# RichExplor/VIL_Fusion

Hardware: AMD Instinct MI355X
Metric: sliding-window solve iters/sec (10 KF, ~5.5k factors) @1/2/4/8 GPU vs CPU (higher is better)
Workload: dtype f64

## Files before the change

### include/vilfusion.h

```cpp
#ifndef VILFUSION_H
#define VILFUSION_H

#include <stdint.h>

#ifdef __cplusplus
extern "C" {
#endif

#define VILF_MAX_FRAMES 11
#define VILF_MAX_FEATURES 1000
#define VILF_PRIOR_MAX_DIM 160
#define VILF_PRIOR_MAX_BLOCKS 24

#define VILF_OK 0
#define VILF_ERR_INVALID_ARGUMENT (-1)
#define VILF_ERR_DEVICE (-2)
#define VILF_ERR_UNSUPPORTED (-3)
#define VILF_ERR_NO_GPU (-4)
#define VILF_SOLVER_ABNORMAL 1

#define VILF_MARGIN_OLD 0
#define VILF_MARGIN_SECOND_NEW 1

#define VILF_TERM_NO_CONVERGENCE 0
// ... 197 lines not shown
    double rel_q[4], rel_t[3];
    int n_edge_ds, n_surf_ds;
    int n_edge_factors[2];
    int n_surf_factors[2];
    int iterations[2];
    double final_cost[2];
    int map_edge_size, map_surf_size;
} vilf_scan2map_result;
int vilf_scan2map_step(vilf_handle *h, const float *edge_xyzi, int n_edge, const float *surf_xyzi, int n_surf,
                       vilf_scan2map_result *res);
int vilf_scan2map_get_map(vilf_handle *h, int which , float *xyzi_out, int capacity, int *n_out);
int vilf_scan2map_set_pose(vilf_handle *h, const double pose_qt[7], const double pose_last_qt[7]);

int vilf_scan2map_batch_create(vilf_handle *h, int n_streams, int cap_scan_edge, int cap_scan_surf, int cap_map_edge, int cap_map_surf);
int vilf_scan2map_batch_init(vilf_handle *h, int stream, const float *edge_xyzi, int n_edge, const float *surf_xyzi, int n_surf,
                             const double *pose_qt, const double *pose_last_qt);
int vilf_scan2map_batch_set_scan(vilf_handle *h, int stream, const float *edge_xyzi, int n_edge, const float *surf_xyzi, int n_surf);
int vilf_scan2map_batch_copy_stream(vilf_handle *h, int src, int dst);
int vilf_scan2map_batch_step(vilf_handle *h, int sync);
int vilf_scan2map_batch_snapshot(vilf_handle *h);
int vilf_scan2map_batch_rewind(vilf_handle *h);
int vilf_scan2map_batch_results(vilf_handle *h, int first, int n, vilf_scan2map_result *res);
int vilf_scan2map_batch_get_map(vilf_handle *h, int stream, int which, float *xyzi_out, int capacity, int *n_out);

int vilf_lidar_extract_features(vilf_handle *h, const float *xyzi, int n_points, int n_scans, double min_range, double max_range,
                                double edge_threshold, float *edge_xyzi_out, int cap_edge, int *n_edge,
                                float *surf_xyzi_out, int cap_surf, int *n_surf);
int vilf_feature_depth(vilf_handle *h, const float *depth_cloud_xyzi, int n_points, const float *features_xyz, int n_features, float *depth_out);
#ifdef __cplusplus
}
#endif
#endif
```

### vil_fusion_amd/csrc/vilf_s2m.hip

```cpp
#include <hip/hip_runtime.h>
#include <cstring>
#include <string.h>
#include <cmath>
#include <climits>
#include <algorithm>
#include <utility>
#include "vilf_sort.hpp"
#include "vilf_internal.hpp"
#include "vilf_device.hpp"

#ifdef VILF_STAMPS
__device__ long long s2m_dbg[9 * 32];
#define S2M_STAMP_WG 1500
#define S2M_STAMP(kid, i, cond) do { if (blockIdx.x == S2M_STAMP_WG && threadIdx.x == 0 && (cond)) s2m_dbg[(kid) * 32 + (i)] = __builtin_readcyclecounter(); } while (0)
extern "C" int vilf_debug_stamps_s2m(long long *out288) { return hipMemcpyFromSymbol(out288, HIP_SYMBOL(s2m_dbg), sizeof(long long) * 9 * 32) == hipSuccess ? 0 : -1; }
#define S2M_ACC_DECL long long acc_t[8] = {0, 0, 0, 0, 0, 0, 0, 0}; long long acc_last = __builtin_readcyclecounter();
#define S2M_ACC(i) do { const long long now_ = __builtin_readcyclecounter(); acc_t[i] += now_ - acc_last; acc_last = now_; } while (0)
#define S2M_ACC_OUT(kid) do { if (blockIdx.x == S2M_STAMP_WG && threadIdx.x == 0) for (int i_ = 0; i_ < 8; i_++) s2m_dbg[(kid) * 32 + 16 + i_] = acc_t[i_]; } while (0)
#else
#define S2M_STAMP(kid, i, cond) do { } while (0)
#define S2M_ACC_DECL
#define S2M_ACC(i) do { } while (0)
#define S2M_ACC_OUT(kid) do { } while (0)
#endif
// ... 717 lines not shown
        if (between)
        for (int jj = hasp ? lower(kp + 1) : 0; jj < jlo;) {
            const unsigned long long lf = T[jj] >> IDXB;
            int f = jj + 1;
            while (f < jlo && (T[f] >> IDXB) == lf) f++;
            o[H + thp(jj) - M] = mu_centroid(ts, jj, f); fixq[atomicAdd(s_fn, 1)] = H + thp(jj) - M;
            jj = f;
        }
        if (tm && !sv) {
            bool any = false;
            for (int b = i + 1; b < nOld; b++) { const float4 r = p[b]; unsigned long long kr; mu_leaf<AXB>(r, inv, cs, kr); if (kr != key) break; if (mu_inside(r, box)) { any = true; break; } }
            if (!any) { o[H + thp(jlo) - M] = mu_centroid(ts, jlo, jup); fixq[atomicAdd(s_fn, 1)] = H + thp(jlo) - M; }
        }
    }
    if (head) {
        float4 s = make_float4(__fadd_rn(0.0f, q.x), __fadd_rn(0.0f, q.y), __fadd_rn(0.0f, q.z), __fadd_rn(0.0f, q.w));
        int cnt = 1;
        for (int b = i + 1; b < nOld; b++) { const float4 r = p[b]; unsigned long long kr; mu_leaf<AXB>(r, inv, cs, kr); if (kr != key) break; if (mu_inside(r, box)) { mu_acc(s, r); cnt++; } }
        for (int jj = jlo; jj < jup; jj++) { mu_acc(s, ts[jj]); cnt++; }
        const float nn = (float)cnt;
        o[H + thp(jlo) - M] = make_float4(s.x / nn, s.y / nn, s.z / nn, s.w / nn); fixq[atomicAdd(s_fn, 1)] = H + thp(jlo) - M;
    }
}
#ifdef MU_WPE
#define MU_LB __launch_bounds__(MU_T, MU_WPE)
#else
#define MU_LB __launch_bounds__(MU_T)
#endif
template <bool BIG>
__global__ MU_LB void b_map_update(CSet map, const int *n_old, const double *pose_all, double half, float inv, int cs, CSet out, unsigned *dir_all, unsigned dtag, int *fix_all, float4 *ts_all, int ts_stride,
                                                       unsigned long long *gT_all, int gT_stride, int lds_lo, int lds_cap, int *gq_all, size_t gq_stride, int *err) {
    constexpr int AXB = BIG ? 16 : 17, IDXB = BIG ? 16 : 13;
    constexpr unsigned long long LOW = (1ULL << IDXB) - 1;
    extern __shared__ unsigned long long s_T[];
    __shared__ int s_w[MU_E][16];
    const int tid = threadIdx.x, lane = tid & 63, wave = tid >> 6, sid = blockIdx.x;
    const int n = map.n[sid], nOld = min(max(n_old[sid], 0), n), nt = n - nOld;
    if (BIG ? nt <= lds_cap : (nt <= lds_lo || nt > lds_cap)) return;
    unsigned long long *T = BIG ? gT_all + (size_t)sid * gT_stride : s_T;
    const float4 *p = map.p + (size_t)sid * map.cap;
    float4 *o = out.p + (size_t)sid * out.cap;
    unsigned *Tdir = dir_all + (size_t)sid * S2B_NBS;
    int *fixq = fix_all + (size_t)sid * out.cap;
    float4 *ts = ts_all + (size_t)sid * ts_stride;
    const double *pose = pose_all + 24 * sid;
    MuBox box;
    box.mnx = (float)(pose[4] - half); box.mny = (float)(pose[5] - half); box.mnz = (float)(pose[6] - half);
    box.mxx = (float)(pose[4] + half); box.mxy = (float)(pose[5] + half); box.mxz = (float)(pose[6] + half);
    int bad = 0;
    [[maybe_unused]] const int skid = nOld > 45000 ? 4 : 5;
    S2M_STAMP(skid, 0, true);

    int P2 = 2;
    while (P2 < nt) P2 <<= 1;
    int myvalid = 0;
    constexpr int NW = MU_T / 64, MU_RADIX = 4096, RK = MU_RADIX / MU_T;
    __shared__ int s_mm[6][NW], s_geo[8];
    bool radix = !BIG && nt <= MU_RADIX && nt <= lds_cap;
    if (radix) {
        unsigned long long kf[RK];
        unsigned vm = 0;
// ... 168 lines not shown
    for (int j = tid; j < ntv; j += MU_T) ts[j] = p[nOld + (int)(T[j] & LOW)];
    __syncthreads();
    int THtot = 0;
    {
        const int C = (P2 + MU_T - 1) / MU_T, j0 = tid * C;
        int cnt = 0;
        for (int j = j0; j < j0 + C && j < ntv; j++) cnt += (j == 0 || (T[j - 1] >> IDXB) != (T[j] >> IDXB)) ? 1 : 0;
        int tot;
        int run = block_excl_scan_nw<MU_T / 64>(cnt, s_w[1], tot);
        THtot = tot;
        unsigned long long prev = (j0 > 0 && j0 <= ntv) ? (T[j0 - 1] >> IDXB) : ~0ULL;
        __syncthreads();
        for (int j = j0; j < j0 + C && j < ntv; j++) {
            const unsigned long long lf = T[j] >> IDXB;
            const int hd = (j == 0 || prev != lf) ? 1 : 0;
            T[j] = (lf << IDXB) | (unsigned long long)run;
            run += hd; prev = lf;
        }
    }
    __syncthreads();
    auto lower = [&](unsigned long long k) { int lo = 0, hi = ntv; while (lo < hi) { const int mid = (lo + hi) >> 1; if ((T[mid] >> IDXB) < k) lo = mid + 1; else hi = mid; } return lo; };
    auto thp = [&](int j) { return j < ntv ? (int)(T[j] & LOW) : THtot; };

    S2M_STAMP(skid, 1, true);
    unsigned long long *s_key = s_T + (BIG ? 0 : lds_cap);
    int *s_te = reinterpret_cast<int *>(s_key + MU_TILE);
    int *gq = gq_all + (size_t)sid * gq_stride;
    __shared__ int s_qn, s_fn, s_jlo;
    __shared__ unsigned long long s_nk;
    if (tid == 0) { s_qn = 0; s_fn = 0; }
    constexpr unsigned long long SVB = 1ULL << 63;
    int carryH = 0, carryM = 0, carryTE = 0, carryJ = 0;
    unsigned long long carryK = 0;
    float4 qn[MU_E], qn2[MU_E];
#pragma unroll
    for (int u = 0; u < MU_E; u++) { qn[u] = p[min(u * MU_T + tid, max(nOld - 1, 0))]; qn2[u] = p[min(MU_TILE + u * MU_T + tid, max(nOld - 1, 0))]; }
    S2M_ACC_DECL
    for (int t0 = 0; t0 < nOld; t0 += MU_TILE) {
        S2M_ACC(0);
        float4 q[MU_E];
        unsigned long long key[MU_E];
        int tb[MU_E], flag[MU_E], incl[MU_E];
        unsigned hm = 0, fm = 0, cm = 0;
#pragma unroll
        for (int u = 0; u < MU_E; u++) { q[u] = qn[u]; qn[u] = qn2[u]; qn2[u] = p[min(t0 + 2 * MU_TILE + u * MU_T + tid, nOld - 1)]; }
#pragma unroll
// ... 118 lines not shown
        for (int k = tid; k < qn; k += MU_T) {
            const int4 e = reinterpret_cast<const int4 *>(gq)[k];
            mu_rare<AXB, IDXB>(e.x & 0x1fffffff, e.y, e.z, (e.x >> 30) & 1, (e.x >> 29) & 1, e.w, nOld, p, o, fixq, &s_fn, ts, T, ntv, THtot, inv, cs, box);
        }
    }
    __syncthreads();
    S2M_STAMP(skid, 3, true);
    int jlast = 0;
    if (nOld > 0) { unsigned long long kl; mu_leaf<AXB>(p[nOld - 1], inv, cs, kl); jlast = lower(kl + 1); }
    for (int jj = jlast + tid; jj < ntv; jj += MU_T) {
        const unsigned long long lf = T[jj] >> IDXB;
        if (jj > jlast && (T[jj - 1] >> IDXB) == lf) continue;
        int e = jj + 1;
        while (e < ntv && (T[e] >> IDXB) == lf) e++;
        o[carryH + thp(jj) - carryM] = mu_centroid(ts, jj, e); fixq[atomicAdd(&s_fn, 1)] = carryH + thp(jj) - carryM;
    }
    S2M_STAMP(skid, 4, true);
#ifdef VILF_STAMPS
    if (blockIdx.x == S2M_STAMP_WG && tid == 0) { s2m_dbg[skid * 32 + 30] = nOld; s2m_dbg[skid * 32 + 29] = nt; s2m_dbg[skid * 32 + 28] = s_qn; }
#endif
    const int n_out = carryH + THtot - carryM;
    if (tid == 0) out.n[sid] = n_out;
    if (bad) atomicOr(err + sid, bad);
    __threadfence_block();
    __syncthreads();
    for (int k = tid; k < s_fn; k += MU_T) {
        const int pos = fixq[k];
        const float4 a = o[pos], ap = o[max(pos - 1, 0)];
        dir_point(Tdir, dtag, pos, n_out, (cm_leaf(a.y, inv) >> cs) & 511, (cm_leaf(a.x, inv) >> cs) & 511, (cm_leaf(ap.y, inv) >> cs) & 511, (cm_leaf(ap.x, inv) >> cs) & 511);
    }
    if (tid == 0 && n_out > 0) {
        const float4 a = o[n_out - 1];
        const int cy = (cm_leaf(a.y, inv) >> cs) & 511, cx = (cm_leaf(a.x, inv) >> cs) & 511;
        for (int c = cx + 1; c <= cx + S2B_DMARGIN; c++) Tdir[dir_slot(cy, c)] = dtag | (unsigned)n_out;
    }
}
__global__ void b_check_order(CSet map, float inv, int cs, int axb, int *flag) {
    const int sid = blockIdx.y, n = map.n[sid];
    const float4 *p = map.p + (size_t)sid * map.cap;
    bool bad = false;
    for (int i = blockIdx.x * blockDim.x + threadIdx.x; i < n; i += gridDim.x * blockDim.x) {
        unsigned long long k, kp = 0;
        const bool ok = axb == 16 ? mu_leaf<16>(p[i], inv, cs, k) : mu_leaf<17>(p[i], inv, cs, k);
        if (i > 0) { if (axb == 16) mu_leaf<16>(p[i - 1], inv, cs, kp); else mu_leaf<17>(p[i - 1], inv, cs, kp); }
        if (!ok || kp > k) bad = true;
    }
    if (bad) atomicOr(flag, 1);
}

#define DIR_PT 8
__global__ void b_dir_build(const float4 *pts_all, const int *n_all, int cap, float inv, int cs, unsigned tag, unsigned *dir_all) {
    const int sid = blockIdx.y, n = min(n_all[sid], cap), i0 = blockIdx.x * DIR_PT * blockDim.x + threadIdx.x;
    if (i0 >= n) return;
    const float4 *p = pts_all + (size_t)sid * cap;
    unsigned *T = dir_all + (size_t)sid * S2B_NBS;
    float2 q[DIR_PT], qp[DIR_PT];
#pragma unroll
    for (int u = 0; u < DIR_PT; u++) {
// ... 659 lines not shown
    r.n_ds[0] = n_ds_e[sid]; r.n_ds[1] = n_ds_s[sid];
    r.do_opt = (n_map_e[sid] > 10 && n_map_s[sid] > 50 && n_ds_e[sid] + n_ds_s[sid] > 0) ? 1 : 0;
    res[sid] = r;
}
__global__ void b_finish(const double *pose_all, const int *n_map_e, const int *n_map_s, const int *err, S2BRes *res, int S) {
    const int sid = blockIdx.x * blockDim.x + threadIdx.x;
    if (sid >= S) return;
    const double *pose = pose_all + 24 * sid;
    for (int k = 0; k < 7; k++) { res[sid].pose[k] = pose[k]; res[sid].prev[k] = pose[16 + k]; }
    res[sid].map_n[0] = n_map_e[sid]; res[sid].map_n[1] = n_map_s[sid];
    res[sid].err = err[sid];
}

struct S2B {
    int S = 0;
    int capScan[2] = {0, 0}, capMap[2] = {0, 0};
    DBuf scan[2], nScan[2], ds[2], nDs[2], map[2], mapAlt[2], nMap[2], tmpB, nTmp, sorted[2], bstart[2], bcnt;
    DBuf nOld, mOld;
    DBuf keys, keys2, vals, vals2, temp, mm, frec, fkind, pose, res, err, bits;
    DBuf map0[2], nMap0[2], pose0, muT, tileHeads;
    DBuf svlist[2];
    DBuf bigmap[2]; std::vector<int> h_big[2];
    DBuf bstartAlt[2], dir0[2], fixq[2];
    bool dir_ok[2] = {false, false}, snap_dir_ok[2] = {false, false};
    unsigned dir_tag[2] = {0, 0}, snap_dir_tag[2] = {0, 0};
    unsigned next_tag() { epoch++; return (epoch % 255u + 1u) << 24; }
    int order_state[2] = {0, 0}, snap_order[2] = {0, 0};
    int cs_cfg[2] = {0, 0};
    int cs_idx[2] = {0, 0};
    bool idx_copy[2] = {false, false};
    unsigned epoch = 0;
    std::vector<int> h_cmn[2], snap_cmn[2];
    bool has_snapshot = false, scan_dirty = true;
    bool snap_live = false;
    void *snap_ptr[2] = {nullptr, nullptr};
    size_t temp_bytes = 0, work_n = 0;
    std::vector<int> h_nScan[2], h_nMap[2];
    std::vector<S2BRes> h_res;
    CSet cs_scan(int w) { return CSet{scan[w].as<float4>(), nScan[w].as<int>(), capScan[w]}; }
    CSet cs_ds(int w) { return CSet{ds[w].as<float4>(), nDs[w].as<int>(), capScan[w]}; }
    CSet cs_map(int w) { return CSet{map[w].as<float4>(), nMap[w].as<int>(), capMap[w]}; }
    CSet cs_tmp(int w) { return CSet{tmpB.as<float4>(), nTmp.as<int>(), capMap[w]}; }
    CSet cs_mapout(int w) { return CSet{mapAlt[w].as<float4>(), nMap[w].as<int>(), capMap[w]}; }
    void release() {
        DBuf *all[] = {&scan[0], &scan[1], &nScan[0], &nScan[1], &ds[0], &ds[1], &nDs[0], &nDs[1], &map[0], &map[1], &mapAlt[0], &mapAlt[1], &nMap[0], &nMap[1], &tmpB, &nTmp, &sorted[0], &sorted[1],
                       &bstart[0], &bstart[1], &bcnt, &nOld, &mOld, &keys, &keys2, &vals, &vals2, &temp, &mm, &frec, &fkind, &pose, &res, &err, &bits,
                       &map0[0], &map0[1], &nMap0[0], &nMap0[1], &pose0, &muT, &tileHeads, &bstartAlt[0], &bstartAlt[1], &dir0[0], &dir0[1], &fixq[0], &fixq[1], &bigmap[0], &bigmap[1]};
        for (DBuf *b : all) b->release();
    }
};

void vilf_s2m_release(vilf_handle *h) {
    for (S2B **pc : {&h->s2m, &h->s2b}) if (*pc) { (*pc)->release(); delete *pc; *pc = nullptr; }
}

static void s2m_prof_mark(vilf_handle *h, int group) {
    hipEvent_t e = vilf_prof_event(h);
    if (!h->s2m_groups.empty()) vilf_prof_span(h, h->s2m_ev.back(), e, &h->s2m_ms[group], &h->s2m_launches[group]);
    h->s2m_ev.push_back(e);
    h->s2m_groups.push_back(group);
}
#define PROF(g) if (h->profiling) s2m_prof_mark(h, (g));
#define GRID2(cap, S) dim3(((cap) + 255) / 256, (S)), dim3(256)
#define GRIDS(S) dim3(((S) + 63) / 64), dim3(64)

static int sbits_of(int S) { int b = 0; while ((1 << b) < S) b++; return b; }
static int s2b_cell_shift(float leaf, double half) {
    int cs = 0;
    while (cs < 15 && ((double)leaf * (1 << cs) < 0.5 || 2.0 * half / ((double)leaf * (1 << cs)) + 2.0 + 2 * S2B_DMARGIN > (double)(1 << S2B_DB))) cs++;
    return cs;
}

static int s2b_reserve(vilf_handle *h, S2B *c, int S, int capScanE, int capScanS, int capMapE, int capMapS) {
    const int wantScan[2] = {std::max(capScanE, 1), std::max(capScanS, 1)}, wantMap[2] = {std::max(capMapE, 1), std::max(capMapS, 1)};
    if (S != c->S) {
        c->release();
        c->S = S; c->capScan[0] = c->capScan[1] = c->capMap[0] = c->capMap[1] = 0; c->work_n = 0; c->has_snapshot = false; c->order_state[0] = c->order_state[1] = 0;
        c->h_big[0].clear(); c->h_big[1].clear();
        if (!c->pose.ensure((size_t)S * 24 * 8) || !c->res.ensure((size_t)S * sizeof(S2BRes)) || !c->err.ensure((size_t)S * 4) || !c->mm.ensure((size_t)S * sizeof(MinMax)) || !c->nTmp.ensure((size_t)S * 4) || !c->bits.ensure(64) || !c->nOld.ensure((size_t)S * 4) || !c->mOld.ensure((size_t)S * 4) || !c->bcnt.ensure((size_t)S * 4)) return VILF_ERR_DEVICE;
        HIPCHECK(h, hipMemsetAsync(c->bcnt.p, 0, (size_t)S * 4, h->stream));
        for (int w = 0; w < 2; w++) {
            if (!c->nScan[w].ensure((size_t)S * 4) || !c->nDs[w].ensure((size_t)S * 4) || !c->nMap[w].ensure((size_t)S * 4) || !c->bstart[w].ensure((size_t)S * S2B_NBS * 4)) return VILF_ERR_DEVICE;
            if (!c->bstartAlt[w].ensure((size_t)S * S2B_NBS * 4)) return VILF_ERR_DEVICE;
            HIPCHECK(h, hipMemsetAsync(c->bstart[w].p, 0, (size_t)S * S2B_NBS * 4, h->stream));
            HIPCHECK(h, hipMemsetAsync(c->bstartAlt[w].p, 0, (size_t)S * S2B_NBS * 4, h->stream));
            c->dir_ok[w] = false;
            c->h_cmn[w].assign(S, 0);
            c->cs_cfg[w] = s2b_cell_shift((float)(w == 0 ? h->opts.edge_leaf_size : h->opts.surf_leaf_size), h->opts.s2m_crop_half);
            HIPCHECK(h, hipMemsetAsync(c->nScan[w].p, 0, (size_t)S * 4, h->stream));
            HIPCHECK(h, hipMemsetAsync(c->nDs[w].p, 0, (size_t)S * 4, h->stream));
            HIPCHECK(h, hipMemsetAsync(c->nMap[w].p, 0, (size_t)S * 4, h->stream));
            c->h_nScan[w].assign(S, 0); c->h_nMap[w].assign(S, 0);
        }
        std::vector<double> ident((size_t)S * 24, 0.0);
        for (int s = 0; s < S; s++) { ident[24 * s + 3] = 1.0; ident[24 * s + 11] = 1.0; ident[24 * s + 19] = 1.0; }
        HIPCHECK(h, hipMemcpyAsync(c->pose.p, ident.data(), ident.size() * 8, hipMemcpyHostToDevice, h->stream));
        HIPCHECK(h, hipMemsetAsync(c->err.p, 0, (size_t)S * 4, h->stream));
        HIPCHECK(h, hipFuncSetAttribute(reinterpret_cast<const void *>(b_scan_voxel<false>), hipFuncAttributeMaxDynamicSharedMemorySize, SV_MAXPTS32 * 8 + 8192));
        HIPCHECK(h, hipFuncSetAttribute(reinterpret_cast<const void *>(b_scan_voxel<true>), hipFuncAttributeMaxDynamicSharedMemorySize, SV_MAXPTS24 * 7 + 8192));
        HIPCHECK(h, hipFuncSetAttribute(reinterpret_cast<const void *>(b_scan_voxel_runs), hipFuncAttributeMaxDynamicSharedMemorySize, (int)sr_lds_bytes(SR_RC)));
        HIPCHECK(h, hipFuncSetAttribute(reinterpret_cast<const void *>(b_map_update<false>), hipFuncAttributeMaxDynamicSharedMemorySize, MU_LDS_TAIL * 8 + MU_TILE * 12));
        HIPCHECK(h, hipStreamSynchronize(h->stream));
        c->h_res.assign(S, S2BRes{});
    }
    bool grew = false;
    for (int w = 0; w < 2; w++) {
        if (wantScan[w] > c->capScan[w]) {
            const int nc = c->capScan[w] ? std::max(wantScan[w], 2 * c->capScan[w]) : wantScan[w];
            if (!c->scan[w].ensure((size_t)S * nc * 16) || !c->ds[w].ensure((size_t)S * nc * 16)) return VILF_ERR_DEVICE;
            c->capScan[w] = nc; grew = true; c->scan_dirty = true;
        }
        if (wantMap[w] > c->capMap[w]) {
            const int oc = c->capMap[w], nc = oc ? std::max(wantMap[w], 2 * oc) : wantMap[w];
            if (nc >= (1 << 24)) { h->err = "scan2map: local-map capacity beyond 2^24 points per stream (directory positions are 24 bits)"; return VILF_ERR_UNSUPPORTED; }
            DBuf nb;
            if (!nb.ensure((size_t)S * nc * 16)) return VILF_ERR_DEVICE;
            if (oc) {
                HIPCHECK(h, hipMemcpy2DAsync(nb.p, (size_t)nc * 16, c->map[w].p, (size_t)oc * 16, (size_t)oc * 16, S, hipMemcpyDeviceToDevice, h->stream));
                HIPCHECK(h, hipStreamSynchronize(h->stream));
            }
            c->map[w].release();
            c->map[w] = nb;
            c->capMap[w] = nc; grew = true; c->has_snapshot = false; c->snap_live = false;
            if (!c->sorted[w].ensure((size_t)S * nc * 16) || !c->mapAlt[w].ensure((size_t)S * nc * 16)) return VILF_ERR_DEVICE;
// ... 181 lines not shown
    bool new_dir_ok[2] = {false, false};
    const unsigned new_tag[2] = {c->next_tag(), c->next_tag()};
    for (int w = 0; w < 2; w++) {
        CSet map = c->cs_map(w), dsw = c->cs_ds(w), tmp = c->cs_tmp(w);
        hipLaunchKernelGGL(b_transform_append, GRID2(dsw.cap, S), 0, h->stream, dsw, d_pose, map, d_err);
        hipLaunchKernelGGL(b_bump, GRIDS(S), 0, h->stream, map, dsw, c->nOld.as<int>(), S);
        PROF(5)
        if (c->has_snapshot && c->snap_live && c->mapAlt[w].p == c->snap_ptr[w]) {
            for (int v = 0; v < 2; v++) {
                if (!c->map0[v].ensure((size_t)S * c->capMap[v] * 16)) return VILF_ERR_DEVICE;
                const bool cur = c->map[v].p == c->snap_ptr[v];
                HIPCHECK(h, hipMemcpyAsync(c->map0[v].p, cur ? c->map[v].p : c->mapAlt[v].p, (size_t)S * c->capMap[v] * 16, hipMemcpyDeviceToDevice, h->stream));
                if (c->snap_dir_ok[v]) {
                    if (!c->dir0[v].ensure((size_t)S * S2B_NBS * 4)) return VILF_ERR_DEVICE;
                    HIPCHECK(h, hipMemcpyAsync(c->dir0[v].p, cur ? c->bstart[v].p : c->bstartAlt[v].p, (size_t)S * S2B_NBS * 4, hipMemcpyDeviceToDevice, h->stream));
                }
            }
            c->snap_live = false;
        }
        if (c->order_state[w] == 1) {
            const int lds_cap = mu_lds_cap(c->capScan[w]), lds_half = std::min(lds_cap, MU_LDS_TAIL / 2);
            int *gq = c->sorted[w].as<int>();
            const size_t gq_stride = (size_t)c->capMap[w] * 4;
            hipLaunchKernelGGL(b_map_update<false>, dim3(S), dim3(MU_T), ((size_t)lds_half * 8 + (size_t)MU_TILE * 12), h->stream, map, c->nOld.as<int>(), d_pose, h->opts.s2m_crop_half, 1.0f / leaf[w], c->cs_cfg[w], c->cs_mapout(w), c->bstartAlt[w].as<unsigned>(), new_tag[w], c->fixq[w].as<int>(),
                               c->tmpB.as<float4>(), c->capScan[w], (unsigned long long *)nullptr, 0, -1, lds_half, gq, gq_stride, d_err);
            if (lds_cap > lds_half)
                hipLaunchKernelGGL(b_map_update<false>, dim3(S), dim3(MU_T), ((size_t)lds_cap * 8 + (size_t)MU_TILE * 12), h->stream, map, c->nOld.as<int>(), d_pose, h->opts.s2m_crop_half, 1.0f / leaf[w], c->cs_cfg[w], c->cs_mapout(w), c->bstartAlt[w].as<unsigned>(), new_tag[w], c->fixq[w].as<int>(),
                                   c->tmpB.as<float4>(), c->capScan[w], (unsigned long long *)nullptr, 0, lds_half, lds_cap, gq, gq_stride, d_err);
            if (c->capScan[w] > lds_cap) {
                int p2 = 2; while (p2 < c->capScan[w]) p2 <<= 1;
                if (!c->muT.ensure((size_t)S * p2 * 8)) return VILF_ERR_DEVICE;
                hipLaunchKernelGGL(b_map_update<true>, dim3(S), dim3(MU_T), (size_t)MU_TILE * 12, h->stream, map, c->nOld.as<int>(), d_pose, h->opts.s2m_crop_half, 1.0f / leaf[w], c->cs_cfg[w], c->cs_mapout(w), c->bstartAlt[w].as<unsigned>(), new_tag[w], c->fixq[w].as<int>(),
                                   c->tmpB.as<float4>(), c->capScan[w], c->muT.as<unsigned long long>(), p2, 0, lds_cap, gq, gq_stride, d_err);
            }
            PROF(7)
            new_dir_ok[w] = true;
        } else {
            hipLaunchKernelGGL(b_crop_compact, dim3(S), dim3(S2B_VT), 0, h->stream, map, d_pose, h->opts.s2m_crop_half, tmp, c->nOld.as<int>(), c->mOld.as<int>());
            PROF(5)
            if ((rc = s2b_voxel(h, c, tmp, leaf[w], c->cs_mapout(w), c->cs_cfg[w])) != VILF_OK) return rc;
        }
        c->order_state[w] = 1;
        std::fill(c->h_cmn[w].begin(), c->h_cmn[w].end(), INT_MAX);
    }
    for (int w = 0; w < 2; w++) {
        std::swap(c->map[w], c->mapAlt[w]); std::swap(c->bstart[w], c->bstartAlt[w]);
        c->dir_ok[w] = new_dir_ok[w]; c->dir_tag[w] = new_tag[w];
    }
    hipLaunchKernelGGL(b_finish, GRIDS(S), 0, h->stream, d_pose, c->nMap[0].as<int>(), c->nMap[1].as<int>(), d_err, d_res, S);
    PROF(6)
    HIPCHECK(h, hipGetLastError());
    if (h->profiling && h->prof_used.size() > 4096) return vilf_prof_flush(h);
    return VILF_OK;
}

static void s2b_fill_result(const S2BRes &r, vilf_scan2map_result *res) {
    std::memset(res, 0, sizeof(*res));
    std::memcpy(res->pose_qt, r.pose, 56);
    res->n_edge_ds = r.n_ds[0]; res->n_surf_ds = r.n_ds[1];
    for (int k = 0; k < 2; k++) { res->n_edge_factors[k] = r.nfe[k]; res->n_surf_factors[k] = r.nfs[k]; res->iterations[k] = r.its[k]; res->final_cost[k] = r.cost[k]; }
// ... 160 lines not shown

extern "C" int vilf_scan2map_batch_init(vilf_handle *h, int stream, const float *e, int ne, const float *s, int ns, const double *pose_qt, const double *pose_last_qt) {
    S2B_CHECK(h, stream)
    if (ne < 0 || ns < 0 || ne > c->capMap[0] || ns > c->capMap[1] || (ne && !e) || (ns && !s)) return VILF_ERR_INVALID_ARGUMENT;
    const float *src[2] = {e, s}; const int nn[2] = {ne, ns};
    int rc;
    std::vector<float> cm[2];
    for (int w = 0; w < 2; w++) {
        if (c->order_state[w] == 1) std::fill(c->h_cmn[w].begin(), c->h_cmn[w].end(), INT_MAX);
        const bool conv = s2b_host_cell_major(src[w], nn[w], (float)(w == 0 ? h->opts.edge_leaf_size : h->opts.surf_leaf_size), c->cs_cfg[w], cm[w]);
        if ((rc = s2b_set_cloud(h, c, c->map[w], c->capMap[w], stream, 0, conv ? cm[w].data() : src[w], nn[w])) != VILF_OK) return rc;
        c->h_cmn[w][stream] = conv ? nn[w] : 0;
        c->h_nMap[w][stream] = nn[w]; c->order_state[w] = 0; c->dir_ok[w] = false;
        HIPCHECK(h, hipMemcpyAsync(c->nMap[w].as<int>() + stream, &c->h_nMap[w][stream], 4, hipMemcpyHostToDevice, h->stream));
    }
    double p[24] = {0};
    p[3] = p[11] = p[19] = 1.0;
    if (pose_qt) for (int k = 0; k < 7; k++) p[k] = p[8 + k] = p[16 + k] = pose_qt[k];
    if (pose_last_qt) for (int k = 0; k < 7; k++) p[8 + k] = pose_last_qt[k];
    HIPCHECK(h, hipMemcpyAsync(c->pose.as<double>() + 24 * (size_t)stream, p, sizeof(p), hipMemcpyHostToDevice, h->stream));
    HIPCHECK(h, hipStreamSynchronize(h->stream));
    return VILF_OK;
}
struct CopyJob { const void *src[8]; void *dst[8]; unsigned long long bytes[8]; int n; };
__global__ void b_copy_regions(CopyJob job) {
    const int r = blockIdx.y;
    if (r >= job.n) return;
    const size_t n4 = job.bytes[r] / 4;
    const bool wide = ((size_t)job.src[r] % 16 == 0) && ((size_t)job.dst[r] % 16 == 0) && n4 % 4 == 0;
    if (wide) { const uint4 *s4 = static_cast<const uint4 *>(job.src[r]); uint4 *d4 = static_cast<uint4 *>(job.dst[r]); for (size_t i = blockIdx.x * (size_t)blockDim.x + threadIdx.x; i < n4 / 4; i += (size_t)gridDim.x * blockDim.x) d4[i] = s4[i]; }
    else { const unsigned *s1 = static_cast<const unsigned *>(job.src[r]); unsigned *d1 = static_cast<unsigned *>(job.dst[r]); for (size_t i = blockIdx.x * (size_t)blockDim.x + threadIdx.x; i < n4; i += (size_t)gridDim.x * blockDim.x) d1[i] = s1[i]; }
}
extern "C" int vilf_scan2map_batch_copy_stream(vilf_handle *h, int src, int dst) {
    S2B_CHECK(h, src)
    if (dst < 0 || dst >= c->S) return VILF_ERR_INVALID_ARGUMENT;
    if (src == dst) return VILF_OK;
    CopyJob job; job.n = 0;
    auto add = [&](const void *s_, void *d_, size_t bytes) { job.src[job.n] = s_; job.dst[job.n] = d_; job.bytes[job.n] = bytes; job.n++; };
    size_t largest = 0;
    for (int w = 0; w < 2; w++) {
        add(c->map[w].as<float4>() + (size_t)src * c->capMap[w], c->map[w].as<float4>() + (size_t)dst * c->capMap[w], (size_t)c->capMap[w] * 16);
        if (c->dir_ok[w]) add(c->bstart[w].as<unsigned>() + (size_t)src * S2B_NBS, c->bstart[w].as<unsigned>() + (size_t)dst * S2B_NBS, (size_t)S2B_NBS * 4);
        add(c->nMap[w].as<int>() + src, c->nMap[w].as<int>() + dst, 4);
        c->h_nMap[w][dst] = c->h_nMap[w][src]; c->h_nScan[w][dst] = c->h_nScan[w][src]; c->h_cmn[w][dst] = c->h_cmn[w][src];
    }
    hipLaunchKernelGGL(b_copy_regions, dim3(64, job.n), dim3(256), 0, h->stream, job);
// ... 91 lines not shown
```

### vil_fusion_amd/lib.py

```python
import ctypes as C
import os
import subprocess
from . import abi

_HERE = os.path.dirname(os.path.abspath(__file__))
CSRC = os.path.join(_HERE, "csrc")
SO_PATH = os.environ.get("VILF_SO") or os.path.join(CSRC, "libvilfusion_hip.so")
_lib = None

EXPORTED = [
    "vilf_default_options", "vilf_create", "vilf_destroy", "vilf_reset", "vilf_last_error", "vilf_version",
    "vilf_window_solve", "vilf_window_solve_group", "vilf_window_marginalize", "vilf_batch_upload", "vilf_batch_solve", "vilf_batch_rewind",
    "vilf_batch_marginalize", "vilf_batch_download", "vilf_batch_download_states", "vilf_batch_summaries", "vilf_synchronize", "vilf_wait_for", "vilf_set_async_upload", "vilf_set_profiling", "vilf_get_profile",
    "vilf_batch_newest_poses_device", "vilf_prior_export", "vilf_prior_import", "vilf_eval_projection", "vilf_eval_imu", "vilf_eval_imu_raw",
    "vilf_eval_lidar_between", "vilf_eval_projection_td", "vilf_eval_prior", "vilf_eval_edge", "vilf_eval_surf", "vilf_pose_plus", "vilf_se3_plus",
    "vilf_imu_preintegrate", "vilf_imu_preintegrate_batch", "vilf_visual_imu_alignment", "vilf_posegraph_optimize", "vilf_scan2map_init", "vilf_scan2map_step", "vilf_scan2map_get_map", "vilf_scan2map_set_pose",
    "vilf_scan2map_batch_create", "vilf_scan2map_batch_init", "vilf_scan2map_batch_set_scan", "vilf_scan2map_batch_step", "vilf_scan2map_batch_snapshot",
    "vilf_scan2map_batch_rewind", "vilf_scan2map_batch_copy_stream", "vilf_scan2map_batch_results", "vilf_scan2map_batch_get_map", "vilf_get_profile_scan2map", "vilf_get_profile_marginalize", "vilf_batch_marginalize_stats", "vilf_get_profile_large_window", "vilf_lidar_extract_features", "vilf_feature_depth",
    "vilf_comm_unique_id", "vilf_comm_create", "vilf_comm_destroy", "vilf_gather_poses", "vilf_gather_poses_handle", "vilf_comm_ranks", "vilf_get_stream", "vilf_comm_last_error",
]


class VilfError(RuntimeError):
    pass


def build(verbose=False):
    subprocess.check_call(["make", "-C", CSRC, "-j4"] + ([] if verbose else ["-s"]))
    res = os.path.join(CSRC, "kernel_resources.json")
    tool = os.path.join(os.path.dirname(_HERE), "tools", "kernel_resources.py")
    if os.path.exists(tool) and (not os.path.exists(res) or os.path.getmtime(res) < os.path.getmtime(SO_PATH)):
        r = subprocess.run(["python3", tool, "__none__"], check=False, stdout=subprocess.PIPE, stderr=subprocess.STDOUT, text=True)
        if r.returncode != 0 or verbose:
            print(f"[vil_fusion_amd.build] tools/kernel_resources.py rc={r.returncode}" + (": " + r.stdout.strip()[-400:] if r.returncode != 0 else ""))
    return SO_PATH


def lib():
    global _lib
    if _lib is not None:
        return _lib
# ... 37 lines not shown
    L.vilf_eval_surf.argtypes = [vp, abi.c_double_p, abi.c_double_p, abi.c_double_p, C.c_double, abi.c_double_p, abi.c_double_p]
    L.vilf_pose_plus.argtypes = [vp, abi.c_double_p, abi.c_double_p, abi.c_double_p]
    L.vilf_se3_plus.argtypes = [vp, abi.c_double_p, abi.c_double_p, abi.c_double_p]
    L.vilf_imu_preintegrate.argtypes = [C.POINTER(abi.ImuNoise), abi.c_double_p, abi.c_double_p, abi.c_double_p, abi.c_double_p, C.c_int,
                                        abi.c_double_p, abi.c_double_p, abi.c_double_p, C.POINTER(abi.ImuPreint)]
    L.vilf_scan2map_init.argtypes = [vp, C.POINTER(C.c_float), C.c_int, C.POINTER(C.c_float), C.c_int]
    L.vilf_scan2map_step.argtypes = [vp, C.POINTER(C.c_float), C.c_int, C.POINTER(C.c_float), C.c_int, C.POINTER(abi.Scan2MapResult)]
    L.vilf_scan2map_get_map.argtypes = [vp, C.c_int, C.POINTER(C.c_float), C.c_int, C.POINTER(C.c_int)]
    L.vilf_scan2map_set_pose.argtypes = [vp, abi.c_double_p, abi.c_double_p]
    fpp = C.POINTER(C.c_float)
    L.vilf_scan2map_batch_create.argtypes = [vp, C.c_int, C.c_int, C.c_int, C.c_int, C.c_int]
    L.vilf_scan2map_batch_init.argtypes = [vp, C.c_int, fpp, C.c_int, fpp, C.c_int, abi.c_double_p, abi.c_double_p]
    L.vilf_scan2map_batch_set_scan.argtypes = [vp, C.c_int, fpp, C.c_int, fpp, C.c_int]
    L.vilf_scan2map_batch_step.argtypes = [vp, C.c_int]
    L.vilf_scan2map_batch_snapshot.argtypes = [vp]
    L.vilf_get_profile_scan2map.argtypes = [vp, C.POINTER(C.c_double), C.POINTER(C.c_long)]
    L.vilf_get_profile_marginalize.argtypes = [vp, C.POINTER(C.c_double), C.POINTER(C.c_long)]
    L.vilf_batch_marginalize_stats.argtypes = [vp, C.POINTER(C.c_int)]
    L.vilf_get_profile_large_window.argtypes = [vp, C.POINTER(C.c_double), C.POINTER(C.c_long)]
    L.vilf_scan2map_batch_rewind.argtypes = [vp]
    L.vilf_scan2map_batch_copy_stream.argtypes = [vp, C.c_int, C.c_int]
    L.vilf_scan2map_batch_results.argtypes = [vp, C.c_int, C.c_int, C.POINTER(abi.Scan2MapResult)]
    L.vilf_scan2map_batch_get_map.argtypes = [vp, C.c_int, C.c_int, fpp, C.c_int, C.POINTER(C.c_int)]
    _lib = L
    return L


def default_options():
    o = abi.Options()
    lib().vilf_default_options(C.byref(o))
    return o
```

Measured before the change: 1.056 million.

## Add fast-path scan-to-map update kernel with fallback to full merge

Adds a FAST variant of the map-update kernel. It locates each new voxel in the old sorted map through the previous directory plus a short walk, then does a streaming wave-level merge that writes kept and inserted points directly. A per-stream flag tells the existing full kernel to skip streams the fast path handled, and to run normally on fallback when order checks fail or the stream is out of range. This targets the scan-to-map lidar step, not the sliding-window solve being measured, so the benchmark is likely unaffected. It adds an extra kernel launch and a test/introspection API.

```diff
diff --git a/include/vilfusion.h b/include/vilfusion.h
--- a/include/vilfusion.h
+++ b/include/vilfusion.h
@@ -243,6 +243,7 @@
 int vilf_scan2map_batch_rewind(vilf_handle *h);
 int vilf_scan2map_batch_results(vilf_handle *h, int first, int n, vilf_scan2map_result *res);
 int vilf_scan2map_batch_get_map(vilf_handle *h, int stream, int which, float *xyzi_out, int capacity, int *n_out);
+int vilf_scan2map_batch_test_map_update(vilf_handle *h, int stream, int which, float *xyzi_out, int capacity, int *n_out, unsigned int *dir_out, int *n_fast);
 
 int vilf_lidar_extract_features(vilf_handle *h, const float *xyzi, int n_points, int n_scans, double min_range, double max_range,
                                 double edge_threshold, float *edge_xyzi_out, int cap_edge, int *n_edge,
diff --git a/vil_fusion_amd/csrc/vilf_s2m.hip b/vil_fusion_amd/csrc/vilf_s2m.hip
--- a/vil_fusion_amd/csrc/vilf_s2m.hip
+++ b/vil_fusion_amd/csrc/vilf_s2m.hip
@@ -763,21 +763,45 @@
         o[H + thp(jlo) - M] = make_float4(s.x / nn, s.y / nn, s.z / nn, s.w / nn); fixq[atomicAdd(s_fn, 1)] = H + thp(jlo) - M;
     }
 }
+__device__ __forceinline__ void mu_dir_fix(const float4 *o, unsigned *Tdir, unsigned dtag, const int *fixq, const int *s_fn, int n_out, float inv, int cs) {
+    const int tid = threadIdx.x;
+    __threadfence_block();
+    __syncthreads();
+    for (int k = tid; k < *s_fn; k += MU_T) {
+        const int pos = fixq[k];
+        const float4 a = o[pos], ap = o[max(pos - 1, 0)];
+        dir_point(Tdir, dtag, pos, n_out, (cm_leaf(a.y, inv) >> cs) & 511, (cm_leaf(a.x, inv) >> cs) & 511, (cm_leaf(ap.y, inv) >> cs) & 511, (cm_leaf(ap.x, inv) >> cs) & 511);
+    }
+    if (tid == 0 && n_out > 0) {
+        const float4 a = o[n_out - 1];
+        const int cy = (cm_leaf(a.y, inv) >> cs) & 511, cx = (cm_leaf(a.x, inv) >> cs) & 511;
+        for (int c = cx + 1; c <= cx + S2B_DMARGIN; c++) Tdir[dir_slot(cy, c)] = dtag | (unsigned)n_out;
+    }
+}
 #ifdef MU_WPE
 #define MU_LB __launch_bounds__(MU_T, MU_WPE)
 #else
 #define MU_LB __launch_bounds__(MU_T)
 #endif
-template <bool BIG>
+#ifndef MU_FE
+#define MU_FE 4
+#endif
+#define MU_WALK 8
+template <bool BIG, bool FAST = false>
 __global__ MU_LB void b_map_update(CSet map, const int *n_old, const double *pose_all, double half, float inv, int cs, CSet out, unsigned *dir_all, unsigned dtag, int *fix_all, float4 *ts_all, int ts_stride,
-                                                       unsigned long long *gT_all, int gT_stride, int lds_lo, int lds_cap, int *gq_all, size_t gq_stride, int *err) {
+                                                       unsigned long long *gT_all, int gT_stride, int lds_lo, int lds_cap, int *gq_all, size_t gq_stride, int *err,
+                                                       int *mflag, const unsigned *odir_all, unsigned otag) {
     constexpr int AXB = BIG ? 16 : 17, IDXB = BIG ? 16 : 13;
     constexpr unsigned long long LOW = (1ULL << IDXB) - 1;
     extern __shared__ unsigned long long s_T[];
     __shared__ int s_w[MU_E][16];
     const int tid = threadIdx.x, lane = tid & 63, wave = tid >> 6, sid = blockIdx.x;
     const int n = map.n[sid], nOld = min(max(n_old[sid], 0), n), nt = n - nOld;
-    if (BIG ? nt <= lds_cap : (nt <= lds_lo || nt > lds_cap)) return;
+    if (BIG ? nt <= lds_cap : (nt <= lds_lo || nt > lds_cap)) {
+        if (FAST && tid == 0) mflag[sid] = 2;
+        return;
+    }
+    if (!FAST && mflag && mflag[sid] == 0) return;
     unsigned long long *T = BIG ? gT_all + (size_t)sid * gT_stride : s_T;
     const float4 *p = map.p + (size_t)sid * map.cap;
     float4 *o = out.p + (size_t)sid * out.cap;
@@ -992,6 +1016,170 @@
     auto lower = [&](unsigned long long k) { int lo = 0, hi = ntv; while (lo < hi) { const int mid = (lo + hi) >> 1; if ((T[mid] >> IDXB) < k) lo = mid + 1; else hi = mid; } return lo; };
     auto thp = [&](int j) { return j < ntv ? (int)(T[j] & LOW) : THtot; };
 
+    if constexpr (FAST) {
+        unsigned *s_evL = reinterpret_cast<unsigned *>(s_T + lds_cap), *s_evJ = s_evL + lds_cap + 1;
+        int *s_evP = reinterpret_cast<int *>(s_T);
+        __shared__ int s_ffn, s_fl;
+        if (tid == 0) { s_ffn = 0; s_fl = 0; }
+        S2M_STAMP(skid, 1, true);
+        auto okey = [&](int x) { unsigned long long kx; mu_leaf<AXB>(p[x], inv, cs, kx); return kx; };
+        auto olower = [&](unsigned long long k, int lo, int hi) { while (lo < hi) { const int mid = (lo + hi) >> 1; if (okey(mid) < k) lo = mid + 1; else hi = mid; } return lo; };
+        for (int j = tid; j < ntv; j += MU_T) {
+            const unsigned long long k = T[j] >> IDXB;
+            if (j > 0 && (T[j - 1] >> IDXB) == k) continue;
+            int L = -1;
+            if (odir_all) {
+                const unsigned v = odir_all[(size_t)sid * S2B_NBS + mu_cid<AXB>(k, cs)];
+                int s = min((int)(v & 0xffffffu), nOld);
+                if ((v & 0xff000000u) == otag && (s == 0 || okey(s - 1) < k)) {
+                    int st = 0;
+                    while (s < nOld && st < MU_WALK && okey(s) < k) { s++; st++; }
+                    L = st < MU_WALK ? s : olower(k, s, nOld);
+                }
+            }
+            if (L < 0) L = olower(k, 0, nOld);
+            const bool mg = L < nOld && okey(L) == k;
+            const int d = (int)(T[j] & LOW);
+            s_evL[d] = (unsigned)L; s_evJ[d] = (unsigned)j | (mg ? 1u << 15 : 0u);
+        }
+        __syncthreads();
+        int nIns;
+        {
+            const int C = (THtot + MU_T - 1) / MU_T, d0 = tid * C, d1 = min(d0 + C, THtot);
+            int cnt = 0;
+            for (int d = d0; d < d1; d++) cnt += (s_evJ[d] >> 15) & 1;
+            int tot;
+            int run = block_excl_scan_nw<NW>(cnt, s_w[0], tot);
+            for (int d = d0; d < d1; d++) { s_evJ[d] |= (unsigned)(d - run) << 16; run += (s_evJ[d] >> 15) & 1; }
+            nIns = THtot - tot;
+            if (tid == 0) { s_evL[THtot] = 0x7fffffffu; s_evJ[THtot] = (unsigned)nIns << 16; }
+        }
+        __syncthreads();
+        S2M_STAMP(skid, 2, true);
+        constexpr int FE = MU_FE, CH = 64 * FE, FT = MU_T * FE;
+        const int last = max(nOld - 1, 0);
+        int fl = bad, keptC = 0, ecur = 0, par = 0;
+        float4 qa[FE], pa;
+#pragma unroll
+        for (int u = 0; u < FE; u++) qa[u] = p[min(wave * CH + u * 64 + lane, last)];
+        pa = p[min(max(wave * CH - 1, 0), last)];
+        auto skip = [&](int e, int bound) {
+            for (;;) {
+                const unsigned long long b = __ballot((int)s_evL[min(e + lane, THtot)] < bound);
+                e += __popcll(b);
+                if (b != ~0ULL) return e;
+            }
+        };
+        const unsigned long long ltm = (1ULL << lane) - 1ULL;
+        for (int t0 = 0; t0 < nOld; t0 += FT) {
+            const int c0 = t0 + wave * CH;
+            float4 q[FE];
+#pragma unroll
+            for (int u = 0; u < FE; u++) { q[u] = qa[u]; qa[u] = p[min(t0 + FT + wave * CH + u * 64 + lane, last)]; }
+            const float4 q0 = pa;
+            pa = p[min(t0 + FT + wave * CH - 1, last)];
+            unsigned long long key[FE], svb[FE], kp[FE];
+            unsigned svm = 0, svpm = 0;
+#pragma unroll
+            for (int u = 0; u < FE; u++) {
+                const bool valid = c0 + u * 64 + lane < nOld, ok = mu_leaf<AXB>(q[u], inv, cs, key[u]);
+                const bool sv = valid && mu_inside(q[u], box);
+                if (valid && !ok) fl = 1;
+                svb[u] = __ballot(sv);
+                if (sv) svm |= 1u << u;
+            }
+            unsigned long long k0;
+            mu_leaf<AXB>(q0, inv, cs, k0);
+            const bool sv0 = mu_inside(q0, box);
+#pragma unroll
+            for (int u = 0; u < FE; u++) {
+                const int i = c0 + u * 64 + lane;
+                const unsigned long long up = __shfl_up(key[u], 1, 64), lw = u == 0 ? k0 : __shfl(key[u > 0 ? u - 1 : 0], 63, 64);
+                kp[u] = lane == 0 ? lw : up;
+                const bool svp = lane == 0 ? (u == 0 ? sv0 : ((svb[u > 0 ? u - 1 : 0] >> 63) & 1)) : ((svb[u] >> (lane - 1)) & 1);
+                if (svp) svpm |= 1u << u;
+                if (i < nOld && i > 0 && kp[u] >= key[u]) fl = 1;
+            }
+            ecur = skip(ecur, c0);
+            const int eend = skip(ecur, min(c0 + CH, nOld));
+            const int rb = (int)(s_evJ[ecur] >> 16);
+            int inl[FE];
+            unsigned atm = 0, mgm = 0;
+#pragma unroll
+            for (int u = 0; u < FE; u++) inl[u] = 0;
+            for (int eb = ecur; eb < eend; eb += 64) {
+                const int ne = min(64, eend - eb), lv = (int)s_evL[min(eb + lane, THtot)], jv = (int)s_evJ[min(eb + lane, THtot)];
+                for (int k = 0; k < ne; k++) {
+                    const int dl = __builtin_amdgcn_readlane(lv, k) - c0 - lane;
+                    if ((__builtin_amdgcn_readlane(jv, k) >> 15) & 1) {
+#pragma unroll
+                        for (int u = 0; u < FE; u++) if (dl == u * 64) mgm |= 1u << u;
+                    } else {
+#pragma unroll
+                        for (int u = 0; u < FE; u++) { inl[u] += dl <= u * 64 ? 1 : 0; if (dl == u * 64) atm |= 1u << u; }
+                    }
+                }
+            }
+            unsigned long long km[FE];
+            int wt = 0;
+#pragma unroll
+            for (int u = 0; u < FE; u++) { km[u] = __ballot(c0 + u * 64 + lane < nOld && (((svm | mgm) >> u) & 1)); wt += __popcll(km[u]); }
+            if (lane == 0) s_w[par][wave] = wt;
+            lds_barrier();
+            int off = 0, tot = 0;
+#pragma unroll
+            for (int k = 0; k < NW; k++) { const int x = s_w[par][k]; if (k < wave) off += x; tot += x; }
+            par ^= 1;
+            int kb[FE], run = keptC + off;
+#pragma unroll
+            for (int u = 0; u < FE; u++) {
+                kb[u] = run + __popcll(km[u] & ltm);
+                run += __popcll(km[u]);
+                const int i = c0 + u * 64 + lane;
+                if (((svm >> u) & 1) && !((mgm >> u) & 1)) {
+                    const int pos = kb[u] + rb + inl[u];
+                    o[pos] = make_float4(__fadd_rn(0.0f, q[u].x), __fadd_rn(0.0f, q[u].y), __fadd_rn(0.0f, q[u].z), __fadd_rn(0.0f, q[u].w));
+                    const bool known = i > 0 && ((svpm >> u) & 1) && !((atm >> u) & 1);
+                    const unsigned cme = mu_cid<AXB>(key[u], cs), cpr = mu_cid<AXB>(kp[u], cs);
+                    if (known && cme == cpr) { }
+                    else if (known && cme == cpr + 1u && (cme & 511u) != 0u) Tdir[cme] = dtag | (unsigned)pos;
+                    else fixq[atomicAdd(&s_ffn, 1)] = pos;
+                }
+            }
+            for (int eb = ecur; eb < eend; eb += 64) {
+                const int e = eb + lane, rel = e < eend ? (int)s_evL[e] - c0 : 0;
+                int v = 0;
+#pragma unroll
+                for (int u = 0; u < FE; u++) { const int x = __shfl(kb[u], rel & 63, 64); if ((rel >> 6) == u) v = x; }
+                if (e < eend) s_evP[e] = v + (int)(s_evJ[e] >> 16);
+            }
+            keptC += tot; ecur = eend;
+        }
+        S2M_STAMP(skid, 3, true);
+        if (fl) s_fl = 1;
+        for (int e = tid; e < THtot; e += MU_T) if ((int)s_evL[e] >= nOld) s_evP[e] = keptC + (int)(s_evJ[e] >> 16);
+        __syncthreads();
+        if (s_fl) { if (tid == 0) mflag[sid] = 1; return; }
+        for (int e = tid; e < THtot; e += MU_T) {
+            const unsigned J = s_evJ[e];
+            const int j0 = (int)(J & 0x7fffu), j1 = e + 1 < THtot ? (int)(s_evJ[e + 1] & 0x7fffu) : ntv, pos = s_evP[e];
+            const float4 qL = p[min((int)s_evL[e], last)];
+            float4 v;
+            if (((J >> 15) & 1) && mu_inside(qL, box)) {
+                float4 s = make_float4(__fadd_rn(0.0f, qL.x), __fadd_rn(0.0f, qL.y), __fadd_rn(0.0f, qL.z), __fadd_rn(0.0f, qL.w));
+                for (int jj = j0; jj < j1; jj++) mu_acc(s, ts[jj]);
+                const float nn = (float)(1 + j1 - j0);
+                v = make_float4(s.x / nn, s.y / nn, s.z / nn, s.w / nn);
+            } else v = mu_centroid(ts, j0, j1);
+            o[pos] = v;
+            fixq[atomicAdd(&s_ffn, 1)] = pos;
+        }
+        const int n_out = keptC + nIns;
+        if (tid == 0) { out.n[sid] = n_out; mflag[sid] = 0; }
+        mu_dir_fix(o, Tdir, dtag, fixq, &s_ffn, n_out, inv, cs);
+        S2M_STAMP(skid, 4, true);
+        return;
+    }
     S2M_STAMP(skid, 1, true);
     unsigned long long *s_key = s_T + (BIG ? 0 : lds_cap);
     int *s_te = reinterpret_cast<int *>(s_key + MU_TILE);
@@ -1156,18 +1344,7 @@
     const int n_out = carryH + THtot - carryM;
     if (tid == 0) out.n[sid] = n_out;
     if (bad) atomicOr(err + sid, bad);
-    __threadfence_block();
-    __syncthreads();
-    for (int k = tid; k < s_fn; k += MU_T) {
-        const int pos = fixq[k];
-        const float4 a = o[pos], ap = o[max(pos - 1, 0)];
-        dir_point(Tdir, dtag, pos, n_out, (cm_leaf(a.y, inv) >> cs) & 511, (cm_leaf(a.x, inv) >> cs) & 511, (cm_leaf(ap.y, inv) >> cs) & 511, (cm_leaf(ap.x, inv) >> cs) & 511);
-    }
-    if (tid == 0 && n_out > 0) {
-        const float4 a = o[n_out - 1];
-        const int cy = (cm_leaf(a.y, inv) >> cs) & 511, cx = (cm_leaf(a.x, inv) >> cs) & 511;
-        for (int c = cx + 1; c <= cx + S2B_DMARGIN; c++) Tdir[dir_slot(cy, c)] = dtag | (unsigned)n_out;
-    }
+    mu_dir_fix(o, Tdir, dtag, fixq, &s_fn, n_out, inv, cs);
 }
 __global__ void b_check_order(CSet map, float inv, int cs, int axb, int *flag) {
     const int sid = blockIdx.y, n = map.n[sid];
@@ -1873,6 +2050,8 @@
     DBuf svlist[2];
     DBuf bigmap[2]; std::vector<int> h_big[2];
     DBuf bstartAlt[2], dir0[2], fixq[2];
+    DBuf muflag;
+    bool mu_fast_ran[2] = {false, false};
     bool dir_ok[2] = {false, false}, snap_dir_ok[2] = {false, false};
     unsigned dir_tag[2] = {0, 0}, snap_dir_tag[2] = {0, 0};
     unsigned next_tag() { epoch++; return (epoch % 255u + 1u) << 24; }
@@ -1896,8 +2075,9 @@
     void release() {
         DBuf *all[] = {&scan[0], &scan[1], &nScan[0], &nScan[1], &ds[0], &ds[1], &nDs[0], &nDs[1], &map[0], &map[1], &mapAlt[0], &mapAlt[1], &nMap[0], &nMap[1], &tmpB, &nTmp, &sorted[0], &sorted[1],
                        &bstart[0], &bstart[1], &bcnt, &nOld, &mOld, &keys, &keys2, &vals, &vals2, &temp, &mm, &frec, &fkind, &pose, &res, &err, &bits,
-                       &map0[0], &map0[1], &nMap0[0], &nMap0[1], &pose0, &muT, &tileHeads, &bstartAlt[0], &bstartAlt[1], &dir0[0], &dir0[1], &fixq[0], &fixq[1], &bigmap[0], &bigmap[1]};
+                       &map0[0], &map0[1], &nMap0[0], &nMap0[1], &pose0, &muT, &tileHeads, &bstartAlt[0], &bstartAlt[1], &dir0[0], &dir0[1], &fixq[0], &fixq[1], &bigmap[0], &bigmap[1], &muflag};
         for (DBuf *b : all) b->release();
+        mu_fast_ran[0] = mu_fast_ran[1] = false;
     }
 };
 
@@ -1915,6 +2095,7 @@
 #define GRID2(cap, S) dim3(((cap) + 255) / 256, (S)), dim3(256)
 #define GRIDS(S) dim3(((S) + 63) / 64), dim3(64)
 
+static size_t mu_fast_lds(int lds_half) { return (size_t)lds_half * 8 + std::max((size_t)MU_TILE * 12, ((size_t)lds_half + 1) * 8); }
 static int sbits_of(int S) { int b = 0; while ((1 << b) < S) b++; return b; }
 static int s2b_cell_shift(float leaf, double half) {
     int cs = 0;
@@ -1928,7 +2109,7 @@
         c->release();
         c->S = S; c->capScan[0] = c->capScan[1] = c->capMap[0] = c->capMap[1] = 0; c->work_n = 0; c->has_snapshot = false; c->order_state[0] = c->order_state[1] = 0;
         c->h_big[0].clear(); c->h_big[1].clear();
-        if (!c->pose.ensure((size_t)S * 24 * 8) || !c->res.ensure((size_t)S * sizeof(S2BRes)) || !c->err.ensure((size_t)S * 4) || !c->mm.ensure((size_t)S * sizeof(MinMax)) || !c->nTmp.ensure((size_t)S * 4) || !c->bits.ensure(64) || !c->nOld.ensure((size_t)S * 4) || !c->mOld.ensure((size_t)S * 4) || !c->bcnt.ensure((size_t)S * 4)) return VILF_ERR_DEVICE;
+        if (!c->pose.ensure((size_t)S * 24 * 8) || !c->res.ensure((size_t)S * sizeof(S2BRes)) || !c->err.ensure((size_t)S * 4) || !c->mm.ensure((size_t)S * sizeof(MinMax)) || !c->nTmp.ensure((size_t)S * 4) || !c->bits.ensure(64) || !c->nOld.ensure((size_t)S * 4) || !c->mOld.ensure((size_t)S * 4) || !c->bcnt.ensure((size_t)S * 4) || !c->muflag.ensure((size_t)S * 2 * 4)) return VILF_ERR_DEVICE;
         HIPCHECK(h, hipMemsetAsync(c->bcnt.p, 0, (size_t)S * 4, h->stream));
         for (int w = 0; w < 2; w++) {
             if (!c->nScan[w].ensure((size_t)S * 4) || !c->nDs[w].ensure((size_t)S * 4) || !c->nMap[w].ensure((size_t)S * 4) || !c->bstart[w].ensure((size_t)S * S2B_NBS * 4)) return VILF_ERR_DEVICE;
@@ -1951,6 +2132,7 @@
         HIPCHECK(h, hipFuncSetAttribute(reinterpret_cast<const void *>(b_scan_voxel<true>), hipFuncAttributeMaxDynamicSharedMemorySize, SV_MAXPTS24 * 7 + 8192));
         HIPCHECK(h, hipFuncSetAttribute(reinterpret_cast<const void *>(b_scan_voxel_runs), hipFuncAttributeMaxDynamicSharedMemorySize, (int)sr_lds_bytes(SR_RC)));
         HIPCHECK(h, hipFuncSetAttribute(reinterpret_cast<const void *>(b_map_update<false>), hipFuncAttributeMaxDynamicSharedMemorySize, MU_LDS_TAIL * 8 + MU_TILE * 12));
+        HIPCHECK(h, hipFuncSetAttribute(reinterpret_cast<const void *>(b_map_update<false, true>), hipFuncAttributeMaxDynamicSharedMemorySize, (int)mu_fast_lds(MU_LDS_TAIL / 2)));
         HIPCHECK(h, hipStreamSynchronize(h->stream));
         c->h_res.assign(S, S2BRes{});
     }
@@ -2178,20 +2360,28 @@
             const int lds_cap = mu_lds_cap(c->capScan[w]), lds_half = std::min(lds_cap, MU_LDS_TAIL / 2);
             int *gq = c->sorted[w].as<int>();
             const size_t gq_stride = (size_t)c->capMap[w] * 4;
+            const char *full_env = std::getenv("VILF_MU_FULL");
+            const bool mu_full = full_env && std::atoi(full_env) != 0;
+            int *mflag = mu_full ? nullptr : c->muflag.as<int>() + (size_t)w * S;
+            if (!mu_full)
+                hipLaunchKernelGGL((b_map_update<false, true>), dim3(S), dim3(MU_T), mu_fast_lds(lds_half), h->stream, map, c->nOld.as<int>(), d_pose, h->opts.s2m_crop_half, 1.0f / leaf[w], c->cs_cfg[w], c->cs_mapout(w), c->bstartAlt[w].as<unsigned>(), new_tag[w], c->fixq[w].as<int>(),
+                                   c->tmpB.as<float4>(), c->capScan[w], (unsigned long long *)nullptr, 0, -1, lds_half, gq, gq_stride, d_err, mflag, c->dir_ok[w] ? c->bstart[w].as<unsigned>() : (const unsigned *)nullptr, c->dir_tag[w]);
+            c->mu_fast_ran[w] = !mu_full;
             hipLaunchKernelGGL(b_map_update<false>, dim3(S), dim3(MU_T), ((size_t)lds_half * 8 + (size_t)MU_TILE * 12), h->stream, map, c->nOld.as<int>(), d_pose, h->opts.s2m_crop_half, 1.0f / leaf[w], c->cs_cfg[w], c->cs_mapout(w), c->bstartAlt[w].as<unsigned>(), new_tag[w], c->fixq[w].as<int>(),
-                               c->tmpB.as<float4>(), c->capScan[w], (unsigned long long *)nullptr, 0, -1, lds_half, gq, gq_stride, d_err);
+                               c->tmpB.as<float4>(), c->capScan[w], (unsigned long long *)nullptr, 0, -1, lds_half, gq, gq_stride, d_err, mflag, (const unsigned *)nullptr, 0u);
             if (lds_cap > lds_half)
                 hipLaunchKernelGGL(b_map_update<false>, dim3(S), dim3(MU_T), ((size_t)lds_cap * 8 + (size_t)MU_TILE * 12), h->stream, map, c->nOld.as<int>(), d_pose, h->opts.s2m_crop_half, 1.0f / leaf[w], c->cs_cfg[w], c->cs_mapout(w), c->bstartAlt[w].as<unsigned>(), new_tag[w], c->fixq[w].as<int>(),
-                                   c->tmpB.as<float4>(), c->capScan[w], (unsigned long long *)nullptr, 0, lds_half, lds_cap, gq, gq_stride, d_err);
+                                   c->tmpB.as<float4>(), c->capScan[w], (unsigned long long *)nullptr, 0, lds_half, lds_cap, gq, gq_stride, d_err, (int *)nullptr, (const unsigned *)nullptr, 0u);
             if (c->capScan[w] > lds_cap) {
                 int p2 = 2; while (p2 < c->capScan[w]) p2 <<= 1;
                 if (!c->muT.ensure((size_t)S * p2 * 8)) return VILF_ERR_DEVICE;
                 hipLaunchKernelGGL(b_map_update<true>, dim3(S), dim3(MU_T), (size_t)MU_TILE * 12, h->stream, map, c->nOld.as<int>(), d_pose, h->opts.s2m_crop_half, 1.0f / leaf[w], c->cs_cfg[w], c->cs_mapout(w), c->bstartAlt[w].as<unsigned>(), new_tag[w], c->fixq[w].as<int>(),
-                                   c->tmpB.as<float4>(), c->capScan[w], c->muT.as<unsigned long long>(), p2, 0, lds_cap, gq, gq_stride, d_err);
+                                   c->tmpB.as<float4>(), c->capScan[w], c->muT.as<unsigned long long>(), p2, 0, lds_cap, gq, gq_stride, d_err, (int *)nullptr, (const unsigned *)nullptr, 0u);
             }
             PROF(7)
             new_dir_ok[w] = true;
         } else {
+            c->mu_fast_ran[w] = false;
             hipLaunchKernelGGL(b_crop_compact, dim3(S), dim3(S2B_VT), 0, h->stream, map, d_pose, h->opts.s2m_crop_half, tmp, c->nOld.as<int>(), c->mOld.as<int>());
             PROF(5)
             if ((rc = s2b_voxel(h, c, tmp, leaf[w], c->cs_mapout(w), c->cs_cfg[w])) != VILF_OK) return rc;
@@ -2398,6 +2588,22 @@
     HIPCHECK(h, hipStreamSynchronize(h->stream));
     return VILF_OK;
 }
+extern "C" int vilf_scan2map_batch_test_map_update(vilf_handle *h, int stream, int which, float *out, int cap, int *n_out, unsigned *dir_out, int *n_fast) {
+    S2B_CHECK(h, stream)
+    if (which < 0 || which > 1 || !n_out || !n_fast || cap < 0 || (cap && !out)) return VILF_ERR_INVALID_ARGUMENT;
+    int n = 0;
+    HIPCHECK(h, vilf_copy_sync(h, &n, c->nMap[which].as<int>() + stream, 4, hipMemcpyDeviceToHost));
+    *n_out = n;
+    if (cap > 0 && n > 0) HIPCHECK(h, vilf_copy_sync(h, out, c->map[which].as<float4>() + (size_t)stream * c->capMap[which], (size_t)std::min(cap, n) * 16, hipMemcpyDeviceToHost));
+    if (dir_out) HIPCHECK(h, vilf_copy_sync(h, dir_out, c->bstart[which].as<unsigned>() + (size_t)stream * S2B_NBS, (size_t)S2B_NBS * 4, hipMemcpyDeviceToHost));
+    *n_fast = 0;
+    if (c->mu_fast_ran[which]) {
+        std::vector<int> f(c->S);
+        HIPCHECK(h, vilf_copy_sync(h, f.data(), c->muflag.as<int>() + (size_t)which * c->S, (size_t)c->S * 4, hipMemcpyDeviceToHost));
+        for (int v : f) *n_fast += v == 0 ? 1 : 0;
+    }
+    return VILF_OK;
+}
 struct CopyJob { const void *src[8]; void *dst[8]; unsigned long long bytes[8]; int n; };
 __global__ void b_copy_regions(CopyJob job) {
     const int r = blockIdx.y;
diff --git a/vil_fusion_amd/lib.py b/vil_fusion_amd/lib.py
--- a/vil_fusion_amd/lib.py
+++ b/vil_fusion_amd/lib.py
@@ -16,7 +16,7 @@
     "vilf_eval_lidar_between", "vilf_eval_projection_td", "vilf_eval_prior", "vilf_eval_edge", "vilf_eval_surf", "vilf_pose_plus", "vilf_se3_plus",
     "vilf_imu_preintegrate", "vilf_imu_preintegrate_batch", "vilf_visual_imu_alignment", "vilf_posegraph_optimize", "vilf_scan2map_init", "vilf_scan2map_step", "vilf_scan2map_get_map", "vilf_scan2map_set_pose",
     "vilf_scan2map_batch_create", "vilf_scan2map_batch_init", "vilf_scan2map_batch_set_scan", "vilf_scan2map_batch_step", "vilf_scan2map_batch_snapshot",
-    "vilf_scan2map_batch_rewind", "vilf_scan2map_batch_copy_stream", "vilf_scan2map_batch_results", "vilf_scan2map_batch_get_map", "vilf_get_profile_scan2map", "vilf_get_profile_marginalize", "vilf_batch_marginalize_stats", "vilf_get_profile_large_window", "vilf_lidar_extract_features", "vilf_feature_depth",
+    "vilf_scan2map_batch_rewind", "vilf_scan2map_batch_copy_stream", "vilf_scan2map_batch_results", "vilf_scan2map_batch_get_map", "vilf_scan2map_batch_test_map_update", "vilf_get_profile_scan2map", "vilf_get_profile_marginalize", "vilf_batch_marginalize_stats", "vilf_get_profile_large_window", "vilf_lidar_extract_features", "vilf_feature_depth",
     "vilf_comm_unique_id", "vilf_comm_create", "vilf_comm_destroy", "vilf_gather_poses", "vilf_gather_poses_handle", "vilf_comm_ranks", "vilf_get_stream", "vilf_comm_last_error",
 ]
 
@@ -100,6 +100,7 @@
     L.vilf_scan2map_batch_copy_stream.argtypes = [vp, C.c_int, C.c_int]
     L.vilf_scan2map_batch_results.argtypes = [vp, C.c_int, C.c_int, C.POINTER(abi.Scan2MapResult)]
     L.vilf_scan2map_batch_get_map.argtypes = [vp, C.c_int, C.c_int, fpp, C.c_int, C.POINTER(C.c_int)]
+    L.vilf_scan2map_batch_test_map_update.argtypes = [vp, C.c_int, C.c_int, fpp, C.c_int, C.POINTER(C.c_int), C.POINTER(C.c_uint), C.POINTER(C.c_int)]
     _lib = L
     return L
 
```

Result: slower. 1.040 million (median of 2 runs) (-1.5%).
